# fryzjergda/DesiRNA

Measured on AMD Instinct MI355X. Metric: replica-folds/sec (MFE+PF, L=200, R=64), higher is better.
Workload: dtype int32 (MFE) + f64 (PF); 1 GPU; BASELINE configs[2]: Eterna100-V1 #69 target (L=200), R=64 uniform-random sequences per GPU, -sf Ed-Epf (MFE fill+traceback, PF inside, eval_structure); replicas_per_gpu=64, replicas_total=64, replicas_on_rank0=64, L=200, exchange_every=100, threads_per_workgroup=1024

## Files before the change

### desirna_amd/csrc/fold_common.hpp

```cpp
#pragma once
#include <stdint.h>

#include "tables.hpp"
#ifdef DRNA_PRIMS_HEADER
#include DRNA_PRIMS_HEADER
#else
#include "gfx950_prims.hpp"
#endif

namespace drna {

constexpr int WAVE = 64;
constexpr int MAXN = 2048;
constexpr int PART_ITEMS = 32;

constexpr int GRES = 28;
enum : int { TW_LIVE = 0, TW_BIRTH = 1, TW_KILL = 2, TW_DEAD = 3 };

#ifndef DRNA_SKIP
#define DRNA_SKIP 0
#endif

enum : int { ST_OK = 0, ST_BAD_CHAR = 1, ST_TRACEBACK = 2, ST_PF_RANGE = 3, ST_SYNC = 4 };

struct Ragged {
  const int* idx = nullptr;
  const int* len = nullptr;
  const int* off = nullptr;
  __device__ int seq_of(int b) const { return idx ? idx[b] : b; }
  __device__ int len_of(int r, int L) const { return len ? len[r] : L; }
  __device__ long long off_of(int r, int L) const { return off ? (long long)off[r] : (long long)r * L; }
};

constexpr int DLAG = 10, KEDGE = DLAG - 5;
constexpr int XP = 224;
struct DualLink {
  int* flagA = nullptr;
  int* flagB = nullptr;
  int32_t* xs = nullptr;
  void* xa = nullptr;
  void* xb = nullptr;
  int base = 0;
  int epoch = 0;
};
__device__ __forceinline__ int dual_base(int epoch, int round) { return (int)((((unsigned)epoch * 8u + (unsigned)round) << 10)); }
__device__ __forceinline__ int dual_done(int epoch) { return (int)((((unsigned)epoch * 8u + 7u) << 10) + 1023u); }
__device__ __forceinline__ bool flag_ge(int v, int target) { return (int)((unsigned)v - (unsigned)target) >= 0; }

__device__ __forceinline__ bool wait_flag_wave(const int* flag, int target) {
  SpinClock clk;
  for (;;) {
    if (flag_ge(__builtin_amdgcn_readfirstlane(ld_agent(flag)), target)) return true;
    if (clk.expired()) return false;
    spin_pause();
  }
}

__device__ __forceinline__ int lane_id() { return threadIdx.x & (WAVE - 1); }
__device__ __forceinline__ int wave_id() { return threadIdx.x >> 6; }

__device__ __forceinline__ int wave_min_i32(int v) {
// ... 284 lines not shown
```

### desirna_amd/csrc/fold_mfe_lds.hpp

```cpp
#pragma once
#include "fold_mfe.hpp"

namespace drna {

constexpr int MFE_FAST_NMAX = 200;
enum : int { E_ALL = 0, E_NEAR = 1, E_FAR = 2, E_COARSE = 3 };
constexpr int GSLOTS = 10;

template <int NT>
struct MfeFastSmem : MfeSmemCore<MFE_FAST_NMAX> {
  static constexpr int NW = NT / WAVE;
  static constexpr int RS = MFE_FAST_NMAX + 2;
  static constexpr int TRI = (MFE_FAST_NMAX - 4) * (MFE_FAST_NMAX - 3) / 2;
  static constexpr int NSLOT = 4 * WAVE;
  static constexpr int NL = MFE_FAST_NMAX + 8;
  int fml[TRI + 8];
  int wring[33 * RS];
  int ciring[32 * RS];
  int dml[4 * RS];
  int hpl[MFE_FAST_NMAX + 2];
  int rowoff[MFE_FAST_NMAX + 2];
  int accG[2][NSLOT], accI[2][NSLOT], accK[2][NSLOT];
  static constexpr int XT_STACK = 0, XT_INT11 = 64, XT_MM1N = 64 + 1024, XT_MM23 = 64 + 1024 + 128;
  int xtab[64 + 1024 + 128 + 128];
// ... 484 lines not shown
  for (int k = tid; k < 1024; k += NT) sm.xtab[SM::XT_INT11 + k] = sm.int11[k] - (((k >> 4) & 7) > 2 ? TermAU : 0);
  for (int k = tid; k < 128; k += NT) {
    sm.xtab[SM::XT_MM1N + k] = sm.mm1n[k] - ((k >> 4) > 2 ? TermAU : 0);
    sm.xtab[SM::XT_MM23 + k] = sm.mm23[k] - ((k >> 4) > 2 ? TermAU : 0);
  }
  for (int j = tid; j <= n && j <= TURN + 1; j += NT) sm.f5[j] = 0;
  if (DUAL) {
    drain_vmem();
    __syncthreads();
    if (tid == 0) st_agent(lk.flagA, lk.base + TURN);
  }
  for (int d = TURN + 1 + wave; d < (DUAL ? min(n, PL_D1) : n); d += NW) mfe_pl_row<false>(sm, T, PL, PLX, ld, n, d, lane, TermAU);
  __syncthreads();
  if (aw < 0) {
    const int d = TURN + 1;
    if (d < n) {
      mfe_prepare_tables<NT>(sm, d, tid, ninio, max_ninio, DUAL ? E_NEAR : E_ALL);
      const int cnt = PL[d * ld + ld - 1];
      if (tid < cnt) { sm.plist[d & 1][tid] = PL[d * ld + tid]; sm.xe[d & 1][tid] = PLX[d * ld + tid]; }
      if (tid == 0) { sm.pcnt[d & 1] = cnt; sm.qhead[0] = 0; sm.qhead[1] = 0; }
    }
  }
  __syncthreads();

  if (aw < 0) {
    int32_t* const xw = reinterpret_cast<int32_t*>(lk.xa);
    int32_t* const xf = xw + (MFE_FAST_NMAX + 2) * XP;
    const int32_t* const xk = reinterpret_cast<const int32_t*>(lk.xb);
    const int32_t* const xi = xk + (MFE_FAST_NMAX + 2) * XP;
    int pfK = INF, pfI = INF, fb_s = 0;
    bool have = false;
    if (DUAL) fb_s = __builtin_amdgcn_readfirstlane(ld_agent(lk.flagB));
    int pw[4] = {0, 0, 0, 0}, px[4] = {0, 0, 0, 0}, pw_cnt = 0;
    auto pl_request = [&](const int dn) {
      const int32_t* row = PL + dn * ld;
      const int32_t* rowx = PLX + dn * ld;
      const bool ag = DUAL && dn >= PL_D1;
      pw_cnt = ag ? ld_agent(row + ld - 1) : row[ld - 1];
      const int nch = (n - dn + WAVE - 1) >> 6;
#pragma unroll
      for (int c = 0; c < 4; c++)
        if (c < nch) {
          const int o = min(lane + c * WAVE, ld - 1);
          pw[c] = ag ? ld_agent(row + o) : row[o];
          px[c] = ag ? ld_agent(rowx + o) : rowx[o];
        }
    };
    if (!sweep_stage && wave == w_pl && TURN + 2 < n) pl_request(TURN + 2);
    for (int k = TURN + 1; k <= n; k++) {
      const int d = k - 1;
      if (DUAL && tid == 0 && d - 2 > TURN) st_agent(lk.flagA, lk.base + d - 2);
      int rqK = INF, rqI = INF, rqF = 0;
      bool rq_have = false, rq_on = false;
      if (DUAL && d > TURN) {
        const int i2 = tid + 1 - ((d + 1) >> 1) - off0;
        rq_have = d + 1 < n && d + 1 >= DUAL_D0 && flag_ge(fb_s, lk.base + d + 1);
        rq_on = rq_have && i2 >= 1 && i2 <= n - d - 1;
        rqK = ld_agent(rq_on ? xk + (d + 1) * XP + i2 : lk.flagB);
        rqI = ld_agent(rq_on ? xi + (d + 1) * XP + i2 : lk.flagB);
        rqF = ld_agent(lk.flagB);
      }
      int fx[4];
      if (!sweep_stage && wave == w_pl) {
        if (k + 1 < n) {
          const int dn = k + 1;
          int* dst = sm.plist[dn & 1];
          int* dxe = sm.xe[dn & 1];
#pragma unroll
          for (int c = 0; c < 4; c++)
            if (lane + c * WAVE < MfeFastSmem<NT>::NL) { dst[lane + c * WAVE] = pw[c]; dxe[lane + c * WAVE] = px[c]; }
          if (lane == 0) { sm.pcnt[dn & 1] = pw_cnt; sm.qhead[dn & 1] = 0; }
        }
        if (k + 2 < n) pl_request(k + 2);
      }
      if (!sweep_q5 && wave == w_q5 && k - 3 >= TURN + 2) {
        const int j = k - 3;
        const int nch = (j - TURN - 1 + WAVE - 1) >> 6;
#pragma unroll
        for (int c = 0; c < 4; c++) {
          const int i = lane + 1 + c * WAVE;
          fx[c] = INF;
          if (c < nch && i <= j - TURN - 1) fx[c] = EXT[j * ld + i];
        }
      }
      if (d > TURN) {
        const int ncell = n - d, sh = d >> 1, par = d & 1;
        const int i = tid + 1 - sh - off0;
        const int dv = as_vector(d), dm1v = as_vector(d - 1);
        int bK = pfK, bI = pfI;
        if (DUAL && d >= DUAL_D0) {
          if (!have) {
            if (!sm.sync_fail && !wait_flag_wave(lk.flagB, lk.base + d)) sm.sync_fail = 1;
            const bool on = i >= 1 && i <= ncell;
            bK = on ? ld_agent(xk + d * XP + i) : INF;
            bI = on ? ld_agent(xi + d * XP + i) : INF;
          }
        }
        if (i >= 1 && i <= ncell) {
          const int aG = sm.accG[par][tid];
          const int aI = DUAL ? min(sm.accI[par][tid], bI) : sm.accI[par][tid];
          const int aK = DUAL ? min(sm.accK[par][tid], bK) : sm.accK[par][tid];
          sm.accG[par][tid] = INF; sm.accI[par][tid] = INF; sm.accK[par][tid] = INF;
          const int j = i + d;
          const int t = pair_type(sm.Sp[i], sm.Sp[j]);
          const int tau = t > 2 ? TermAU : 0;
          int c = INF, info = 0, cb = INF;
          if (t) {
            const int ij = t * 16 + sm.S[i + 1] * 4 + sm.S[j - 1];
            c = mfe_hairpin_e(sm, T, sm.hpl[dm1v], i, j, t);
            c = min(c, aI);
            c = min(c, aG + sm.mmI[ij]);
            const int dml = sm.dml[((d - 2) & 3) * RS + i + 1];
            if (dml < HALF)
              c = min(c, dml + MLclosing + MLintern + tau + sm.mmM[rtype_of(t) * 16 + sm.S[j - 1] * 4 + sm.S[i + 1]]);
            if (c >= HALF) c = INF;
            info = (rtype_of(t) << 4) | (sm.S[j + 1] << 2) | sm.S[i - 1];
            cb = c < INF ? c + tau : INF;
          }
          sm.wring[(d & 31) * RS + i] = cb * 256 + info;
          sm.ciring[(d & 31) * RS + i] = c < INF ? c + sm.mmI[info] : INF;
          {
            Wc[d * ld + i] = c * 256 + info;
            EXT[j * ld + i] = c < INF ? c + tau + mfe_extstem(sm, t, i, j, n) : INF;
          }
          int f = INF;
          if (d - 1 > TURN) {
            const int ro1 = sm.rowoff[dm1v];
            const int fa = sm.fml[ro1 + i], fb = sm.fml[ro1 + i - 1];
            if (fa < HALF) f = fa + MLbase;
            if (fb < HALF) f = min(f, fb + MLbase);
          }
          if (c < INF) f = min(f, c + MLintern + tau + sm.mmM[t * 16 + sm.S[i - 1] * 4 + sm.S[j + 1]]);
          const int dec = aK >= HALF ? INF : aK;
          sm.dml[(d & 3) * RS + i] = dec;
          const int fv = min(f, dec);
          sm.fml[sm.rowoff[dv] + i - 1] = fv;
          if (DUAL) {
            st_agent(xw + d * XP + i, cb * 256 + info);
            st_agent(xf + d * XP + i, fv);
          }
        }
      }
      if (k + 1 < n) {
        const bool outer_idle = NB > 3 && (d >> 1) + off0 >= WAVE;
        const int we = outer_idle ? NB - 1 : w_et;
        if (wave == we) mfe_prepare_etab(sm, k + 1, lane, DUAL ? E_NEAR : E_ALL);
      }
      if (!sweep_q5 && wave == w_q5 && k - 3 >= TURN + 2) {
        const int j = k - 3;
        int m = INF;
#pragma unroll
        for (int c = 0; c < 4; c++) {
          const int i = lane + 1 + c * WAVE;
          if (i <= j - TURN - 1 && fx[c] < HALF) m = min(m, sm.f5[i - 1] + fx[c]);
        }
        m = wave_min_i32_lane63(m);
        const int prev = sm.f5[j - 1];
        if (lane == WAVE - 1) sm.f5[j] = prev < m ? prev : m;
      }
      bool stored = false;
      if (d > TURN) { const int i_ = tid + 1 - (d >> 1) - off0; stored = __ballot(i_ >= 1 && i_ <= n - d) != 0ull; }
      if (DUAL && d > TURN) {
        pfK = rq_on ? rqK : INF; pfI = rq_on ? rqI : INF;
        have = rq_have;
        fb_s = __builtin_amdgcn_readfirstlane(rqF);
      }
      if (stored) stores_in_flight<DUAL ? 4 : 2>(); else stores_in_flight<0>();
      lds_barrier();
    }
  } else {
    int GE[TSL_M], GO[TSL_M];
#pragma unroll
    for (int r = 0; r < TSL_M; r++) { GE[r] = INF; if (TWO_PAR) GO[r] = INF; }
    const int e_bulge1 = keep_i32(T.bulge[1]), e_int23 = keep_i32(T.interior[5] + ninio);
    const int blk_ord = my_tb < 0 ? 0 : my_tb == 0 ? 0 : my_tb == NBT - 1 ? min(1, NBT - 1) : my_tb + 1;
    const int n_free = NA - (TWO_PAR ? 2 : 4) * NBT;
    auto item_rank_of = [&](const int par) -> int {
      if (TWO_PAR) return aw;
      if (my_tb < 0) return aw - 4 * NBT;
      const bool rests = !((my_pm >> par) & 1);
      return n_free + (rests ? 0 : 2 * NBT) + 2 * blk_ord + my_sig;
    };

    int sw[4] = {0, 0, 0, 0}, sx[4] = {0, 0, 0, 0}, sw_cnt = 0;
    auto st_request = [&](const int dn) {
      const int32_t* row = PL + dn * ld;
      const int32_t* rowx = PLX + dn * ld;
      const bool ag = DUAL && dn >= PL_D1;
      sw_cnt = ag ? ld_agent(row + ld - 1) : row[ld - 1];
      const int nch = (n - dn + WAVE - 1) >> 6;
#pragma unroll
      for (int c = 0; c < 4; c++)
        if (c < nch) {
          const int o = min(lane + c * WAVE, ld - 1);
          sw[c] = ag ? ld_agent(row + o) : row[o];
          sx[c] = ag ? ld_agent(rowx + o) : rowx[o];
        }
    };
    if (stager && ((my_pm >> ((TURN + 1) & 1)) & 1) && TURN + 2 < n) st_request(TURN + 2);
    for (int k = TURN + 1; k <= n; k++) {
      if (q5er && !((my_pm >> (k & 1)) & 1) && k - 3 >= TURN + 2) {
        const int j = k - 3;
        const int nch = (j - TURN - 1 + WAVE - 1) >> 6;
        int fx[4];
#pragma unroll
        for (int c = 0; c < 4; c++) {
          const int i = lane + 1 + c * WAVE;
          fx[c] = INF;
          if (c < nch && i <= j - TURN - 1) fx[c] = EXT[j * ld + i];
        }
        int m = INF;
#pragma unroll
        for (int c = 0; c < 4; c++) {
          const int i = lane + 1 + c * WAVE;
          if (i <= j - TURN - 1 && fx[c] < HALF) m = min(m, sm.f5[i - 1] + fx[c]);
        }
        m = wave_min_i32_lane63(m);
        const int prev = sm.f5[j - 1];
        if (lane == WAVE - 1) sm.f5[j] = prev < m ? prev : m;
      }
// ... 145 lines not shown
```

### desirna_amd/csrc/fold_pf_lds.hpp

```cpp
#pragma once
#include <cstddef>
#include "eval_structure.hpp"
#include "fold_pf.hpp"

namespace drna {

constexpr int PF_FAST_NMAX = 200;
constexpr int PGSLOTS = 10;
constexpr int PNG = 3;
constexpr int TSL = 14;

template <int NT>
struct PfFastSmem {
  static constexpr int NW = NT / WAVE;
  static constexpr int RS = PF_FAST_NMAX + 2;
  static constexpr int NSLOT = 4 * WAVE;
  static constexpr int NL = PF_FAST_NMAX + 8;
  double qbi[32 * RS];
  double dring[4 * RS];
  double qm1row[2][RS];
  double urow[2][RS];
  double hpw[PF_FAST_NMAX + 2];
  double q5[PF_FAST_NMAX + 2];
  double partG[2][2][NSLOT];
// ... 106 lines not shown
  for (int q = Q1 - 1; q >= Q0; q--) {
    const int s = 4 + SIG + 2 * q;
    if (s > 30) continue;
    G[q] = q > 0 ? fma3_f64(a[q - Q0] + b[q - Q0], c[q - Q0].x, G[q - 1]) : (a[q - Q0] + b[q - Q0]) * c[q - Q0].x;
    acc += G[q] * c[q - Q0].y;
  }
}

template <class SM, int SIG>
__device__ __forceinline__ double pf_tower2_step(const SM& sm, double (&G)[TSL], int dv, int i8) {
  const int cbase = as_vector((int)(reinterpret_cast<const char*>(&sm.twc[0][0]) - reinterpret_cast<const char*>(sm.qbi)));
  double acc0 = 0.0, acc1 = 0.0, acc2 = 0.0;
  pf_tower2_part<SM, SIG, 9, 14>(sm, G, dv, i8, cbase, acc0);
  pf_tower2_part<SM, SIG, 4, 9>(sm, G, dv, i8, cbase, acc1);
  pf_tower2_part<SM, SIG, 0, 4>(sm, G, dv, i8, cbase, acc2);
  return (acc0 + acc1) + acc2;
}


#ifndef DRNA_PKE
#define DRNA_PKE 5
#endif
constexpr int PKE = DRNA_PKE;
constexpr int KT_NL = PKE + 3;
constexpr int KT_U = (2 * KT_NL + 3) / 4;
constexpr int KT_BMIN = (12 + 2 * PKE + 3) / 4;
constexpr int KT_D0 = 4 * KT_BMIN - 3;
constexpr int KT_MF = (4 * ((PF_FAST_NMAX - 1) / 4) - 11 - 2 * PKE + 15) / 16;
constexpr int KT_DEPTH = 3;
static_assert(PKE >= 4, "a tile's operands must be final when the first of its four steps comes");

__device__ __forceinline__ void kt_near_counts(int i, int d, int& nl, int& nh) {
  const int j = i + d, a = (i - 1) >> 2, c = (j - 1) >> 2, tot = max(d - 2 * TURN - 2, 0);
  if (c - a >= KT_BMIN) { nl = 4 * a + 4 + PKE - i; nh = j - 4 * c - 1 + PKE; }
  else { nl = min(tot, KT_NL); nh = tot - nl; }
}
__device__ __forceinline__ bool kt_has_far(int i, int d) { return ((i + d - 1) >> 2) - ((i - 1) >> 2) >= KT_BMIN; }

template <typename RS>
__device__ __forceinline__ void k_near_row(RS rs, int tab8, int ld, int d, int i, int row, double& v0, double& v1) {
  int nl0, nh0, nl1, nh1;
  kt_near_counts(i, d, nl0, nh0);
  kt_near_counts(i + 1, d, nl1, nh1);
  f64x2 a[KT_U], c[KT_U];
#pragma unroll
  for (int u = 0; u < KT_U; u++) {
    const int s = row + 4 * u, y = s - KT_NL;
    const bool low = s < KT_NL;
    const bool ok0 = low ? s < nl0 : y < nh0, ok1 = low ? s < nl1 : y < nh1;
    int tt = low ? TURN + 1 + s : d - TURN - 2 - y;
    tt = (ok0 || ok1) ? tt : TURN + 1;
    a[u] = buf_load_f64x2(rs, (tt * ld + i) * 8, 0);
    c[u] = buf_load_f64x2(rs, tab8 + ((d - tt - 1) * ld + i + tt + 1) * 8, 0);
    if (!ok0) a[u].x = 0.0;
    if (!ok1) a[u].y = 0.0;
  }
  double p0 = 0.0, p1 = 0.0, q0 = 0.0, q1 = 0.0;
#pragma unroll
  for (int u = 0; u < KT_U; u++) {
    if (u & 1) { p1 = fma(a[u].x, c[u].x, p1); q1 = fma(a[u].y, c[u].y, q1); }
    else { p0 = fma(a[u].x, c[u].x, p0); q0 = fma(a[u].y, c[u].y, q0); }
  }
  v0 = p0 + p1; v1 = q0 + q1;
}

constexpr int KT_PRE = 3;
struct KTile {
  double al, bl, av[KT_PRE], bv[KT_PRE];
  int vA, vB;
  int a, c, last;
  bool mask_last;
};
template <bool SC1, typename RS>
__device__ __forceinline__ void k_tile_issue(RS rs, int tab8, int ld, int n, int a, int B, int lane, KTile& t) {
  const int c = a + B, m_lo = 4 * a + 9 + PKE, m_hi = 4 * c - 3 - PKE;
  const int last = __builtin_amdgcn_readfirstlane((m_hi - m_lo + 16) >> 4) - 1;
  const int q = lane & 3, moff = (lane & 12) + (lane >> 4);
  const int i = 4 * a + 1 + q, jc = min(4 * c + 1 + q, n);
  const int sA = 16 * ld * 8, sB = 16 * (ld - 1) * 8;
  const int m0 = m_lo + moff, ml = min(m0 + 16 * last, m_hi);
  const int vA = (i - (1 + i) * ld + m0 * ld) * 8;
  const int vB = tab8 + (jc * ld - (m0 + 16 * last) * (ld - 1)) * 8;
  const int vAl = (i - (1 + i) * ld + ml * ld) * 8, vBl = tab8 + (jc * ld - ml * (ld - 1)) * 8;
  t.a = a; t.c = c; t.last = last; t.mask_last = m0 + 16 * last > m_hi; t.vA = vA; t.vB = vB;
#pragma unroll
  for (int u = 0; u < KT_PRE; u++) {
    if (u < last) {
      t.av[u] = SC1 ? buf_load_f64_aux(rs, vA, u * sA) : buf_load_f64(rs, vA, u * sA);
      t.bv[u] = SC1 ? buf_load_f64_aux(rs, vB, (last - u) * sB) : buf_load_f64(rs, vB, (last - u) * sB);
    }
  }
  t.al = SC1 ? buf_load_f64_aux(rs, vAl, 0) : buf_load_f64(rs, vAl, 0);
  t.bl = SC1 ? buf_load_f64_aux(rs, vBl, 0) : buf_load_f64(rs, vBl, 0);
}
template <bool SC1, typename RS, typename ST>
__device__ __forceinline__ void k_tile_finish(RS rs, int ld, const KTile& t, int n, int lane, ST store) {
  const int sA = 16 * ld * 8, sB = 16 * (ld - 1) * 8, last = t.last;
  double acc0 = 0.0, acc1 = 0.0;
#pragma unroll
  for (int u = 0; u < KT_PRE; u++) {
    if (u < last) {
      if (u & 1) acc1 = mfma_f64_4x4x4_4b(t.av[u], t.bv[u], acc1);
      else acc0 = mfma_f64_4x4x4_4b(t.av[u], t.bv[u], acc0);
    }
  }
#pragma unroll
  for (int u0 = KT_PRE; u0 < KT_MF - 1; u0 += KT_DEPTH) {
    if (u0 < last) {
// ... 54 lines not shown
  const int ld = A.ld, tid = threadIdx.x, lane = lane_id();
  const int wave = __builtin_amdgcn_readfirstlane(wave_id());
  double* base = A.ws + (long long)r * A.ws_stride;
  const long long tab = (long long)ld * ld;
  double* DFAR = base + 5 * tab;
  const auto rsX = __builtin_amdgcn_make_buffer_rsrc((void*)base, (short)0, (int)(2 * tab * 8), 0x00020000);
  const int* flagA = A.hflags + (long long)r * 64;
  int* flagB = A.hflags + (long long)r * 64 + 32;
  int* ctl = reinterpret_cast<int*>(&sm);
  if (tid == 0) ctl[0] = 0;
  if (EV.n_targets > 0) {
    constexpr int NEV = NW < 8 ? NW : 8;
    EvalSmem* es = reinterpret_cast<EvalSmem*>(ctl + 32);
    if (wave < NEV)
      for (int k = wave; k < EV.n_targets; k += NEV) eval_one(es[wave], EV, r, k, lane);
  }
  {
    const char* seq = A.seqs + A.rg.off_of(r, n);
    for (int k = tid; k < n; k += NT) { const int c = enc_nt(seq[k]); sm.S[k + 1] = (unsigned char)(c < 0 ? 0 : c); }
    if (tid == 0) { sm.S[0] = 0; sm.S[n + 1] = 0; }
    __syncthreads();
    int32_t* PL = reinterpret_cast<int32_t*>(base + 4 * tab);
    for (int d = PFL_D1 + wave; d < n; d += NW) pf_pl_row<true>(sm, PL, ld, n, d, lane);
    drain_vmem();
  }
  __syncthreads();
  if (tid == 0) st_agent(flagB, A.hbase + KT_D0 - 1);
  const int Bmax = (n - 1) >> 2;
  for (int B = KT_BMIN; B <= Bmax; B++) {
    if (wave == 0) {
      int seen = 0;
      const bool ok = strip_wait(flagA, A.hbase, 4 * B - 5 - PKE, seen);
      if (lane == 0 && (!ok || seen == A.hbase + STRIP_DONE)) ctl[0] = 1;
    }
    __syncthreads();
    if (ctl[0]) break;
    if (!(DRNA_SKIP & 8))
      for (int a = wave; a <= Bmax - B; a += NW) {
        KTile t;
        k_tile_issue<true>(rsX, (int)tab * 8, ld, n, a, B, lane, t);
        k_tile_finish<true>(rsX, ld, t, n, lane, [&](int d, int i, double v) { st_agent(&DFAR[d * ld + i], v); });
      }
    drain_vmem();
    __syncthreads();
    if (tid == 0) st_agent(flagB, A.hbase + (B == Bmax ? n : 4 * B));
  }
}

template <int NT, bool TILES = true>
__device__ __forceinline__ void pf_lds_body(PfFastSmem<NT>& sm, PfArgs A, const EvalArgs& EV, int bx_in = -1, int helper_in = -1) {
  constexpr int NW = NT / WAVE;
  constexpr int RS = PfFastSmem<NT>::RS;
  const PfTables& T = *A.T;
  const bool hm = A.helper != 0;
  const int bx = bx_in >= 0 ? bx_in : hm ? blockIdx.x >> 1 : blockIdx.x;
  const bool is_helper = hm && (helper_in >= 0 ? helper_in != 0 : (blockIdx.x & 1) != 0);
  const int r = A.rg.seq_of(bx);
  A.L = A.rg.len_of(r, A.L);
  const int n = A.L, ld = A.ld;
  if (is_helper) {
    if (A.helper == 2) return;
    pf_kfar_helper<NT>(A, EV, sm, r, n);
    return;
  }
  const int tid = threadIdx.x, lane = lane_id();
  const int wave = __builtin_amdgcn_readfirstlane(wave_id());

  double* base = A.ws + (long long)r * A.ws_stride;
  const long long tab = (long long)ld * ld;
  double* QM = base + 2 * tab;
  double* QM1 = base + 3 * tab;
  int32_t* PL = reinterpret_cast<int32_t*>(base + 4 * tab);
  double* QEXT = base + 6 * tab;

  const double eTau = T.TermAU, eMLc = T.MLclosing, eMLi = T.MLintern;
  const double b1 = A.eMLb[1], sc1 = A.scale[1], sc2 = A.scale[2];

  stage_energy_tables<NT>(sm, T, tid);
  for (int k = tid; k < 128; k += NT) {
    const double inv = 1.0 / T.mmI[k];
    sm.rinv[k] = inv;
    sm.rbul[k] = ((k >> 4) > 2 ? eTau : 1.0) * inv;
    sm.r1n[k] = T.mm1n[k] * inv;
    sm.r23[k] = T.mm23[k] * inv;
  }
  for (int k = tid; k <= n; k += NT) sm.hpw[k] = A.hp_w[k];
  for (int t = tid; t < 36; t += NT) {
    sm.eWt[t][0] = t >= 2 && t <= 30 ? T.bulge[t] * A.scale[t + 2] : 0.0;
    sm.eWt[t][1] = t >= 4 && t <= 30 ? T.interior[t] * T.eninio[t - 2] * A.scale[t + 2] : 0.0;
  }
  if (tid == 0) {
    sm.xc[0] = T.bulge[1] * A.scale[3]; sm.xc[1] = T.interior[5] * T.eninio[1] * A.scale[7];
    sm.xc[2] = A.scale[4]; sm.xc[3] = A.scale[5]; sm.xc[4] = A.scale[6];
    sm.xc[8] = eTau; sm.xc[9] = eMLc; sm.xc[10] = eMLi; sm.xc[11] = b1; sm.xc[12] = sc2;
  }
  for (int k = tid; k < 32; k += NT) {
    sm.twc[k][0] = k >= 4 && k <= 30 ? T.eninio[k - 4] : 0.0;
    sm.twc[k][1] = k >= 6 && k <= 30 ? T.interior[k] * A.scale[k + 2] : 0.0;
  }
  for (int k = tid; k < 4 * RS; k += NT) sm.dring[k] = 0.0;
  for (int k = tid; k < 32 * RS; k += NT) { sm.qbi[k] = 0.0; sm.info[k] = 0; }
  for (int k = tid; k < 2 * RS; k += NT) { (&sm.qm1row[0][0])[k] = 0.0; (&sm.urow[0][0])[k] = 0.0; }
  for (int k = tid; k < 2 * 2 * PfFastSmem<NT>::NSLOT; k += NT) (&sm.partG[0][0][0])[k] = 0.0;
  for (int k = tid; k < 2 * 4 * PfFastSmem<NT>::NSLOT; k += NT) (&sm.partK[0][0][0])[k] = 0.0;
  for (int k = tid; k < 2 * PfFastSmem<NT>::NSLOT; k += NT) (&sm.accE[0][0])[k] = 0.0;
  for (int k = tid; k < 6 * PfFastSmem<NT>::NSLOT; k += NT) (&sm.accX[0][0][0])[k] = 0.0;
  if (tid == 0) sm.q5[0] = 1.0;
// ... 10 lines not shown

  const int NB = (n + WAVE - 1) / WAVE;
  const int off0 = (NB * WAVE - n) / 2;
  const int aw = wave - NB;
  constexpr bool TWO_PAR = NT < 1024;
  const int nT = n - 10, NBT = nT > 0 ? (nT + WAVE - 1) / WAVE : 0;
  const int T0 = max(0, off0 + 5 - (NBT * WAVE - nT) / 2);
  int my_tb = -1, my_sig = 0, my_pm = 0;
  if (aw >= 0) {
    if (TWO_PAR) { if (aw < 2 * NBT) { my_tb = aw >> 1; my_sig = aw & 1; my_pm = 3; } }
    else if (aw < 4 * NBT) { my_tb = aw >> 2; const int x = (aw + my_tb) & 3; my_sig = x & 1; my_pm = 1 << (x >> 1); }
  }
  const int w_pl = NB > 2 ? 2 : 0, w_q5 = NB - 1;

  if (aw < 0) {
    const int d = TURN + 1;
    if (d < n) {
      const int cnt = PL[d * ld + ld - 1];
      if (tid < cnt) sm.plist[d & 1][tid] = PL[d * ld + tid];
      if (tid == 0) { sm.pcnt[d & 1] = cnt; sm.qhead[0] = 0; sm.qhead[1] = 0; sm.qtile[0] = 0; sm.qtile[1] = 0; }
    }
  }
  __syncthreads();


  const auto rsQ = __builtin_amdgcn_make_buffer_rsrc((void*)QM, (short)0, (int)(2 * tab * 8), 0x00020000);


  double* XQM = base, *XQM1 = base + tab, *DFAR = base + 5 * tab;
  int* flagA = hm ? A.hflags + (long long)r * 64 : nullptr;
  const int* flagB = hm ? A.hflags + (long long)r * 64 + 32 : nullptr;
  double dfar_cur = 0.0, dfar_next = 0.0;
  int fb_last = 0;
  bool helper_lost = false, pl_seen = false;
  auto run_items = [&](const int d) {
    const int ncell = n - d, sh = d >> 1, par = d & 1;
    const int slot0 = sh + off0 - 1;
    const int pcnt = __builtin_amdgcn_readfirstlane(sm.pcnt[par]);
    const int nblk = (ncell + 31) >> 5;
    const int nK = ((DRNA_SKIP & 8) || d < 2 * TURN + 3) ? 0 : nblk;
    const int nE = (DRNA_SKIP & 2) ? 0 : (pcnt + 3) >> 2, nX = (DRNA_SKIP & 4) ? 0 : 3 * ((pcnt + WAVE - 1) / WAVE);
    const int nItems = __builtin_amdgcn_readfirstlane(nK + nE + nX);
    for (int it0 = queue_pop(&sm.qhead[par], lane); it0 < nItems; it0 = queue_pop(&sm.qhead[par], lane)) {
      const int it = it0 < nX ? nK + nE + it0 : it0 - nX;
      if (it < nK) {
        const int blk = it, cl = lane & 15, row = lane >> 4;
        int i = (blk << 5) + 2 * cl + 1;
        const bool act0 = i <= ncell, act1 = i + 1 <= ncell;
        i = act0 ? i : 1;
        double v0, v1;
        k_near_row(rsQ, (int)tab * 8, ld, d, i, row, v0, v1);
        if (act0) sm.partK[par][row][i + slot0] = v0;
        if (act1) sm.partK[par][row][i + 1 + slot0] = v1;
      } else if (it < nK + nE) {
        const int q = 4 * (it - nK) + (lane >> 4);
        const int pe = sm.plist[par][q < pcnt ? q : pcnt - 1];
        const int i0 = pe & 255, ij = pe >> 8;
        const int tA = (lane & 15) + 2, tBr = tA + 16, tB = tBr > 30 ? 30 : tBr;
        const f64x2 wA = *reinterpret_cast<const f64x2*>(&sm.eWt[tA][0]), wB = *reinterpret_cast<const f64x2*>(&sm.eWt[tBr][0]);
        const int oA = ((d - 2 - tA) & 31) * RS + i0, oB = ((d - 2 - tB) & 31) * RS + i0;
        const double a1 = sm.qbi[oA + 1], a2 = sm.qbi[oA + 2], a3 = sm.qbi[oA + tA], a4 = sm.qbi[oA + tA + 1];
        const double b1_ = sm.qbi[oB + 1], b2_ = sm.qbi[oB + 2], b3_ = sm.qbi[oB + tB], b4_ = sm.qbi[oB + tB + 1];
        const int fa1 = sm.info[oA + 1], fa2 = sm.info[oA + 2], fa3 = sm.info[oA + tA], fa4 = sm.info[oA + tA + 1];
        const int fb1 = sm.info[oB + 1], fb2 = sm.info[oB + 2], fb3 = sm.info[oB + tB], fb4 = sm.info[oB + tB + 1];
        const double ra1 = sm.rbul[fa1], ra4 = sm.rbul[fa4], ra2 = sm.r1n[fa2], ra3 = sm.r1n[fa3];
        const double rb1 = sm.rbul[fb1], rb4 = sm.rbul[fb4], rb2 = sm.r1n[fb2], rb3 = sm.r1n[fb3];
        const double bul = (a1 * ra1 + a4 * ra4) * wA.x + (b1_ * rb1 + b4_ * rb4) * wB.x;
        const double one = (a2 * ra2 + a3 * ra3) * wA.y + (b2_ * rb2 + b3_ * rb3) * wB.y;
        double v = bul * ((ij >> 4) > 2 ? sm.xc[as_vector(8)] : 1.0) + one * sm.mm1n[ij];
        v = dpp_add_f64<0x111, 0xF>(v);
        v = dpp_add_f64<0x112, 0xF>(v);
        v = dpp_add_f64<0x114, 0xF>(v);
        v = dpp_add_f64<0x118, 0xF>(v);
        if ((lane & 15) == 15 && q < pcnt) sm.accE[par][i0 + slot0] = v;
      } else {
        const int xi = it - nK - nE;
        const int ch = xi / 3, grp = xi - 3 * ch;
        const int q = ch * WAVE + lane;
        const int pe = sm.plist[par][q < pcnt ? q : pcnt - 1];
        const int i = pe & 255, cxv = pe >> 8, t = cxv >> 4, si1 = (cxv >> 2) & 3, sj1 = cxv & 3;
        double sum;
        if (grp == 0) {
          double w[4];
          int f[4];
#pragma unroll
          for (int shp = 0; shp < 4; shp++) {
            const int u1 = shp >> 1, u2 = shp == 1 || shp == 3 ? 1 : 0;
            const int dp = d - 2 - u1 - u2;
            const int off = (dp & 31) * RS + 1 + u1 + i;
            w[shp] = dp > TURN ? sm.qbi[off] : 0.0;
            f[shp] = dp > TURN ? sm.info[off] : 0;
          }
          sum = w[0] * sm.rinv[f[0]] * sm.stack[t * 8 + (f[0] >> 4)] * sm.xc[as_vector(12)];
          sum += (w[1] * sm.rinv[f[1]] * sm.stack[t * 8 + (f[1] >> 4)] + w[2] * sm.rinv[f[2]] * sm.stack[t * 8 + (f[2] >> 4)]) * sm.xc[as_vector(0)];
          sum += w[3] * sm.rinv[f[3]] * sm.int11[(t * 8 + (f[3] >> 4)) * 16 + si1 * 4 + sj1] * sm.xc[as_vector(2)];
        } else if (grp == 1) {
          const int dpa = d - 5, dpb = d - 6;
          const int oa = (dpa & 31) * RS + 2 + i, ob = (dpa & 31) * RS + 3 + i, oc = (dpb & 31) * RS + 3 + i;
          const double wa = dpa > TURN ? sm.qbi[oa] : 0.0, wb = dpa > TURN ? sm.qbi[ob] : 0.0, wc = dpb > TURN ? sm.qbi[oc] : 0.0;
          const int fa = dpa > TURN ? sm.info[oa] : 0, fb = dpa > TURN ? sm.info[ob] : 0, fc = dpb > TURN ? sm.info[oc] : 0;
          const double ga = T.int21[(t * 8 + (fa >> 4)) * 64 + si1 * 16 + ((fa >> 2) & 3) * 4 + sj1];
          const double gb = T.int21[((fb >> 4) * 8 + t) * 64 + ((fb >> 2) & 3) * 16 + si1 * 4 + (fb & 3)];
          const double gc = T.int22[(t * 8 + (fc >> 4)) * 256 + si1 * 64 + (fc & 3) * 16 + ((fc >> 2) & 3) * 4 + sj1];
          sum = (wa * sm.rinv[fa] * ga + wb * sm.rinv[fb] * gb) * sm.xc[as_vector(3)] + wc * sm.rinv[fc] * gc * sm.xc[as_vector(4)];
        } else {
          const int dp = d - 7;
          const int oa = (dp & 31) * RS + 3 + i, ob = (dp & 31) * RS + 4 + i;
          const double wa = dp > TURN ? sm.qbi[oa] : 0.0, wb = dp > TURN ? sm.qbi[ob] : 0.0;
          const int fa = dp > TURN ? sm.info[oa] : 0, fb = dp > TURN ? sm.info[ob] : 0;
          sum = (wa * sm.r23[fa] + wb * sm.r23[fb]) * sm.mm23[cxv] * sm.xc[as_vector(1)];
        }
        if (q < pcnt) sm.accX[par][grp][i + slot0] = sum;
      }
    }
  };

  auto run_tiles = [&](const int d) {
    const int Bmax = (n - 1) >> 2, Bt = ((d + 3) >> 2) + 1, ph = (d + 3) & 3;
    if (!TILES || (DRNA_SKIP & 8) || hm || Bt < KT_BMIN || Bt > Bmax) return;
    const int cnt = Bmax - Bt + 1, per = (cnt + 3) >> 2, a0 = ph * per;
    const int nT = __builtin_amdgcn_readfirstlane(max(0, min(cnt, a0 + per) - a0));
    for (int it = queue_pop(&sm.qtile[d & 1], lane); it < nT; it = queue_pop(&sm.qtile[d & 1], lane)) {
      KTile t;
      k_tile_issue<false>(rsQ, (int)tab * 8, ld, n, a0 + it, Bt, lane, t);
      k_tile_finish<false>(rsQ, ld, t, n, lane, [&](int dd, int ii, double v) { DFAR[dd * ld + ii] = v; });
    }
  };

  if (aw < 0) {
    double fTau = sm.xc[as_vector(8)], fMLc = sm.xc[as_vector(9)], fMLi = sm.xc[as_vector(10)], fb1 = sm.xc[as_vector(11)], fsc2 = sm.xc[as_vector(12)];
    int pl_cnt = 0, pl0 = 0, pl1 = 0, pl2 = 0, pl3 = 0;
    auto pl_request = [&](const int dn) {
      const int32_t* row = PL + dn * ld;
      if (hm && dn >= PFL_D1) {
        if (!pl_seen) {
          int seen = 0;
          if (!helper_lost && !flag_ge(fb_last, A.hbase + KT_D0 - 1) && !strip_wait(flagB, A.hbase, KT_D0 - 1, seen)) { sm.flag = 2; helper_lost = true; }
          pl_seen = true;
        }
        pl_cnt = ld_agent(row + ld - 1);
        pl0 = ld_agent(row + lane); pl1 = ld_agent(row + lane + WAVE); pl2 = ld_agent(row + lane + 2 * WAVE);
        pl3 = ld_agent(row + min(lane + 3 * WAVE, ld - 1));
      } else {
        pl_cnt = row[ld - 1];
        pl0 = row[lane]; pl1 = row[lane + WAVE]; pl2 = row[lane + 2 * WAVE]; pl3 = row[min(lane + 3 * WAVE, ld - 1)];
      }
    };
    if (wave == w_pl && TURN + 2 < n) pl_request(TURN + 2);
    for (int k = TURN + 1; k <= n; k++) {
      const int d = k - 1;
      if (wave == w_pl) {
        if (k + 1 < n) {
          int* dst = sm.plist[(k + 1) & 1];
          dst[lane] = pl0; dst[lane + WAVE] = pl1; dst[lane + 2 * WAVE] = pl2;
          if (lane + 3 * WAVE < PfFastSmem<NT>::NL) dst[lane + 3 * WAVE] = pl3;
          if (lane == 0) { sm.pcnt[(k + 1) & 1] = pl_cnt; sm.qhead[(k + 1) & 1] = 0; sm.qtile[(k + 1) & 1] = 0; }
        }
        if (k + 2 < n) pl_request(k + 2);
      }
      const bool job_q5 = wave == w_q5 && k - 3 >= TURN + 2;
      double qx0 = 0.0, qx1 = 0.0, qx2 = 0.0, qx3 = 0.0;
      if (job_q5) {
        const int j = k - 3, top = j - TURN - 1;
        const double* col = QEXT + j * ld;
        qx0 = lane + 1 <= top ? col[lane + 1] : 0.0;
        qx1 = lane + 1 + WAVE <= top ? col[lane + 1 + WAVE] : 0.0;
        qx2 = lane + 1 + 2 * WAVE <= top ? col[lane + 1 + 2 * WAVE] : 0.0;
        qx3 = lane + 1 + 3 * WAVE <= top ? col[lane + 1 + 3 * WAVE] : 0.0;
      }
      int f_req = 0;
      double d_req = 0.0;
      dfar_cur = dfar_next;
      if (hm) {
        if (tid == 0 && k - 2 > TURN) st_agent(flagA, A.hbase + (k - 2));
        f_req = ld_agent(flagB);
        if (k >= KT_D0 && k < n && !helper_lost && !flag_ge(fb_last, A.hbase + k)) {
          int seen = 0;
          if (!strip_wait(flagB, A.hbase, k, seen)) { sm.flag = 2; helper_lost = true; }
        }
      }
      if (k >= KT_D0 && k < n) {
        const int ic = tid + 1 - (k >> 1) - off0;
        if (ic >= 1 && ic <= n - k && kt_has_far(ic, k)) d_req = hm ? ld_agent(&DFAR[k * ld + ic]) : DFAR[k * ld + ic];
      }
      if (d > TURN) {
        const int ncell = n - d, sh = d >> 1, par = d & 1;
        const int i = tid + 1 - sh - off0;
        if (i >= 1 && i <= ncell) {
          const int j = i + d;
          const int si = sm.S[i], sj = sm.S[j], si1 = sm.S[i + 1],
                    sj1 = sm.S[j - 1], sim = sm.S[i - 1], sjp = sm.S[j + 1];
          const double aG = d >= 10 ? sm.partG[par][0][tid] + sm.partG[par][1][tid] : 0.0;
          const double aKn = d >= 2 * TURN + 3 ? (sm.partK[par][0][tid] + sm.partK[par][1][tid]) + (sm.partK[par][2][tid] + sm.partK[par][3][tid]) : 0.0;
          const double aK = aKn + dfar_cur;
          const int t = pair_type(si, sj);
          const double cTau = fTau, cMLc = fMLc, cMLi = fMLi, cb1 = fb1, csc2 = fsc2;
          const double tau = t > 2 ? cTau : 1.0;
          const int ij = t * 16 + si1 * 4 + sj1, rt = rtype_of(t);
          const int info = t ? (rt << 4) | (sjp << 2) | sim : 0;
          const double aE = sm.accE[par][tid], aX = (sm.accX[par][0][tid] + sm.accX[par][1][tid]) + sm.accX[par][2][tid];
          const double wH = sm.mmH[ij], wI = sm.mmI[ij], wMc = sm.mmM[rt * 16 + sj1 * 4 + si1], wInfo = sm.mmI[info];
          const double dprev = sm.dring[((d - 2) & 3) * RS + i + 1];
          const int ex = t * 16 + sim * 4 + sjp;
          const double wExt = sm.mmExt[ex], wMs = sm.mmM[ex], w5 = sm.d5[t * 4 + sim], w3 = sm.d3[t * 4 + sjp];
          const int pp = (d - 1) & 1;
          const double m1p = sm.qm1row[pp][i], m1q = sm.qm1row[pp][i + 1], up = sm.urow[pp][i + 1];
          double qb = 0.0;
          if (t) {
            const int u = d - 1;
            double hp;
            if (u == 3 || u == 4 || u == 6) {
              int code = 0;
              const int len = u + 2;
              for (int q = 0; q < len; q++) code |= sm.S[i + q] << (2 * q);
              hp = -1.0;
              if (u == 3) { for (int q = 0; q < T.n_tri; q++) if (T.tri_code[q] == code) hp = T.tri_w[q] * A.scale[u + 2]; if (hp < 0.0) hp = sm.hpw[u] * tau; }
              else if (u == 4) { for (int q = 0; q < T.n_tetra; q++) if (T.tetra_code[q] == code) hp = T.tetra_w[q] * A.scale[u + 2]; }
              else { for (int q = 0; q < T.n_hexa; q++) if (T.hexa_code[q] == code) hp = T.hexa_w[q] * A.scale[u + 2]; }
              if (hp < 0.0) hp = sm.hpw[u] * wH;
            } else {
              hp = sm.hpw[u] * wH;
            }
            qb = hp + aE + aX + aG * wI;
            qb += dprev * cMLc * cMLi * tau * wMc * csc2;
          }
          sm.qbi[(d & 31) * RS + i] = qb * wInfo;
          sm.info[(d & 31) * RS + i] = (unsigned char)info;
          const double me = (i > 1 && j < n) ? wExt : i > 1 ? w5 : j < n ? w3 : 1.0;
          const double mm = (i > 1 && j < n) ? wMs : i > 1 ? w5 : j < n ? w3 : 1.0;
          const double ext = t ? qb * tau * me : 0.0, stem = t ? qb * cMLi * tau * mm : 0.0;
          const double m1 = m1p * cb1 + stem;
          const double U = cb1 * (m1q + up);
          sm.qm1row[par][i] = m1;
          sm.urow[par][i] = U;
          sm.dring[(d & 3) * RS + i] = aK;
          {
            QEXT[j * ld + i] = ext;
            QM1[d * ld + i] = m1;
            QM[d * ld + i] = m1 + aK + U;
            if (hm) { st_agent(&XQM1[d * ld + i], m1); st_agent(&XQM[d * ld + i], m1 + aK + U); }
          }
        }
      }
      if (job_q5) {
        const int j = k - 3, top = j - TURN - 1;
        double sq = 0.0;
        if (lane + 1 <= top) sq += sm.q5[lane] * qx0;
        if (lane + 1 + WAVE <= top) sq += sm.q5[lane + WAVE] * qx1;
        if (lane + 1 + 2 * WAVE <= top) sq += sm.q5[lane + 2 * WAVE] * qx2;
        if (lane + 1 + 3 * WAVE <= top) sq += sm.q5[lane + 3 * WAVE] * qx3;
        sq = wave_total_f64_lane63(sq);
        if (lane == WAVE - 1) sm.q5[j] = sm.q5[j - 1] * sc1 + sq;
      }
      if (k < n) run_items(k);
      dfar_next = d_req;
      if (hm) fb_last = __builtin_amdgcn_readfirstlane(f_req);
      __syncthreads();
    }
  } else {
    double GE[TSL], GO[TSL];
#pragma unroll
    for (int q = 0; q < TSL; q++) { GE[q] = 0.0; if (TWO_PAR) GO[q] = 0.0; }
    for (int k = TURN + 1; k <= n; k++) {
      if (k < n) {
        const int d = k;
        const int ncell = n - d, sh = d >> 1, par = d & 1;
        const int lo = sh + off0, hi = ncell + sh + off0 - 1;

        if (!(DRNA_SKIP & 1) && ((my_pm >> par) & 1) && d >= 10) {
          const int blo = T0 + my_tb * WAVE;
          int i = blo + lane + 1 - sh - off0;
          i = i < 1 ? 1 : (i > ncell ? ncell : i);
          const int dv = as_vector(d + 30), i8 = i * 8;
          if (blo <= hi && blo + WAVE - 1 >= lo) {
            double accG = 0.0;
            if constexpr (TWO_PAR) {
              if (par) accG = my_sig ? pf_tower2_step<PfFastSmem<NT>, 1>(sm, GO, dv, i8) : pf_tower2_step<PfFastSmem<NT>, 0>(sm, GO, dv, i8);
            }
            if (!TWO_PAR || !par) accG = my_sig ? pf_tower2_step<PfFastSmem<NT>, 1>(sm, GE, dv, i8) : pf_tower2_step<PfFastSmem<NT>, 0>(sm, GE, dv, i8);
            sm.partG[par][my_sig][T0 + my_tb * WAVE + lane] = accG;
          }
        }
        run_tiles(d);
        run_items(d);
      }
      __syncthreads();
    }
  }

  const int jq0 = max(TURN + 2, n - 2);
  if (NW >= 3) {
    if (wave < 3 && jq0 + wave <= n) {
      const int j = jq0 + wave;
      double sq = 0.0;
      for (int i = lane + 1; i <= j - TURN - 1; i += WAVE) sq += sm.q5[i - 1] * QEXT[j * ld + i];
      sq = wave_total_f64_lane63(sq);
      if (lane == WAVE - 1) sm.xc[13 + wave] = sq;
    }
    __syncthreads();
    if (tid == 0)
      for (int j = jq0; j <= n; j++) sm.q5[j] = sm.q5[j - 1] * sc1 + sm.xc[13 + j - jq0];
    __syncthreads();
  } else if (wave == 0) {
    for (int j = jq0; j <= n; j++) pf_q5_column<NT>(sm, QEXT, ld, j, lane, sc1);
  }
  if (wave == 0) {
    if (lane == 0) {
      const double Z = sm.q5[n];
      if (!(Z > 0.0) || !(Z < 1.0e300)) {
        A.status[r] = ST_PF_RANGE;
// ... 24 lines not shown
```

Baseline: 151,900 replica-folds/s.

## Make global stores unconditional and replace full barriers with LDS-only barriers in helper mode

In both the MFE and PF LDS kernels, the per-diagonal global stores in helper/dual mode now happen unconditionally outside the cell-active branch: inactive lanes write to a dummy index 0, so the stores are issued uniformly. Asm-based 'take_over' fences pin prefetched agent loads so the compiler schedules them early. Full __syncthreads plus store waits are replaced by an LDS-only barrier, with a single vmem drain on the last iteration. In the PF kernel, helper mode is forced on for the non-tiled path and the helper flag is signalled one diagonal later. The MFE hairpin energy for longer loops is simplified to a table lookup. All of this is meant to let global-memory traffic overlap with compute across diagonals, at the risk of ordering bugs and of writing garbage values to slot 0.

```diff
diff --git a/desirna_amd/csrc/fold_common.hpp b/desirna_amd/csrc/fold_common.hpp
--- a/desirna_amd/csrc/fold_common.hpp
+++ b/desirna_amd/csrc/fold_common.hpp
@@ -7,6 +7,20 @@
 #else
 #include "gfx950_prims.hpp"
 #endif
+
+namespace drna {
+#ifdef DRNA_PRIMS_HEADER
+inline void issue_fence() {}
+template <typename T> inline void take_over(T&) {}
+template <typename T, typename U> inline void take_over(T&, U&) {}
+template <typename T, typename U, typename V> inline void take_over(T&, U&, V&) {}
+#else
+__device__ __forceinline__ void issue_fence() { __builtin_amdgcn_sched_barrier(0); }
+template <typename T> __device__ __forceinline__ void take_over(T& x) { asm volatile("" : "+v"(x)); }
+template <typename T, typename U> __device__ __forceinline__ void take_over(T& x, U& y) { asm volatile("" : "+v"(x), "+v"(y)); }
+template <typename T, typename U, typename V> __device__ __forceinline__ void take_over(T& x, U& y, V& z) { asm volatile("" : "+v"(x), "+v"(y), "+v"(z)); }
+#endif
+}
 
 namespace drna {
 
diff --git a/desirna_amd/csrc/fold_mfe_lds.hpp b/desirna_amd/csrc/fold_mfe_lds.hpp
--- a/desirna_amd/csrc/fold_mfe_lds.hpp
+++ b/desirna_amd/csrc/fold_mfe_lds.hpp
@@ -560,7 +560,7 @@
       if (DUAL && tid == 0 && d - 2 > TURN) st_agent(lk.flagA, lk.base + d - 2);
       int rqK = INF, rqI = INF, rqF = 0;
       bool rq_have = false, rq_on = false;
-      if (DUAL && d > TURN) {
+      if (DUAL) {
         const int i2 = tid + 1 - ((d + 1) >> 1) - off0;
         rq_have = d + 1 < n && d + 1 >= DUAL_D0 && flag_ge(fb_s, lk.base + d + 1);
         rq_on = rq_have && i2 >= 1 && i2 <= n - d - 1;
@@ -591,6 +591,7 @@
           if (c < nch && i <= j - TURN - 1) fx[c] = EXT[j * ld + i];
         }
       }
+      int o_wc = 0, o_ext = 0, o_xw = 0, o_xf = 0;
       if (d > TURN) {
         const int ncell = n - d, sh = d >> 1, par = d & 1;
         const int i = tid + 1 - sh - off0;
@@ -602,6 +603,7 @@
             const bool on = i >= 1 && i <= ncell;
             bK = on ? ld_agent(xk + d * XP + i) : INF;
             bI = on ? ld_agent(xi + d * XP + i) : INF;
+            take_over(bK, bI);
           }
         }
         if (i >= 1 && i <= ncell) {
@@ -615,7 +617,8 @@
           int c = INF, info = 0, cb = INF;
           if (t) {
             const int ij = t * 16 + sm.S[i + 1] * 4 + sm.S[j - 1];
-            c = mfe_hairpin_e(sm, T, sm.hpl[dm1v], i, j, t);
+            if (d - 1 > 6) c = sm.hpl[dm1v] + sm.mmH[ij];
+            else { c = mfe_hairpin_e(sm, T, sm.hpl[dm1v], i, j, t); take_over(c); }
             c = min(c, aI);
             c = min(c, aG + sm.mmI[ij]);
             const int dml = sm.dml[((d - 2) & 3) * RS + i + 1];
@@ -628,8 +631,9 @@
           sm.wring[(d & 31) * RS + i] = cb * 256 + info;
           sm.ciring[(d & 31) * RS + i] = c < INF ? c + sm.mmI[info] : INF;
           {
-            Wc[d * ld + i] = c * 256 + info;
-            EXT[j * ld + i] = c < INF ? c + tau + mfe_extstem(sm, t, i, j, n) : INF;
+            const int wc = c * 256 + info, ext = c < INF ? c + tau + mfe_extstem(sm, t, i, j, n) : INF;
+            if (DUAL) { o_wc = wc; o_ext = ext; }
+            else { Wc[d * ld + i] = wc; EXT[j * ld + i] = ext; }
           }
           int f = INF;
           if (d - 1 > TURN) {
@@ -643,11 +647,17 @@
           sm.dml[(d & 3) * RS + i] = dec;
           const int fv = min(f, dec);
           sm.fml[sm.rowoff[dv] + i - 1] = fv;
-          if (DUAL) {
-            st_agent(xw + d * XP + i, cb * 256 + info);
-            st_agent(xf + d * XP + i, fv);
-          }
-        }
+          if (DUAL) { o_xw = cb * 256 + info; o_xf = fv; }
+        }
+      }
+      if (DUAL) {
+        const int i = tid + 1 - (d >> 1) - off0;
+        const bool on = d > TURN && i >= 1 && i <= n - d;
+        const int is = on ? i : 0, js = on ? i + d : d;
+        Wc[d * ld + is] = o_wc;
+        EXT[js * ld + is] = o_ext;
+        st_agent(xw + d * XP + is, o_xw);
+        st_agent(xf + d * XP + is, o_xf);
       }
       if (k + 1 < n) {
         const bool outer_idle = NB > 3 && (d >> 1) + off0 >= WAVE;
@@ -666,14 +676,17 @@
         const int prev = sm.f5[j - 1];
         if (lane == WAVE - 1) sm.f5[j] = prev < m ? prev : m;
       }
-      bool stored = false;
-      if (d > TURN) { const int i_ = tid + 1 - (d >> 1) - off0; stored = __ballot(i_ >= 1 && i_ <= n - d) != 0ull; }
-      if (DUAL && d > TURN) {
+      if (DUAL) {
+        take_over(rqK, rqI, rqF);
         pfK = rq_on ? rqK : INF; pfI = rq_on ? rqI : INF;
         have = rq_have;
         fb_s = __builtin_amdgcn_readfirstlane(rqF);
-      }
-      if (stored) stores_in_flight<DUAL ? 4 : 2>(); else stores_in_flight<0>();
+      } else {
+        bool stored = false;
+        if (d > TURN) { const int i_ = tid + 1 - (d >> 1) - off0; stored = __ballot(i_ >= 1 && i_ <= n - d) != 0ull; }
+        if (stored) stores_in_flight<2>(); else stores_in_flight<0>();
+      }
+      if (k == n) drain_vmem();
       lds_barrier();
     }
   } else {
diff --git a/desirna_amd/csrc/fold_pf_lds.hpp b/desirna_amd/csrc/fold_pf_lds.hpp
--- a/desirna_amd/csrc/fold_pf_lds.hpp
+++ b/desirna_amd/csrc/fold_pf_lds.hpp
@@ -182,8 +182,14 @@
     tt = (ok0 || ok1) ? tt : TURN + 1;
     a[u] = buf_load_f64x2(rs, (tt * ld + i) * 8, 0);
     c[u] = buf_load_f64x2(rs, tab8 + ((d - tt - 1) * ld + i + tt + 1) * 8, 0);
-    if (!ok0) a[u].x = 0.0;
-    if (!ok1) a[u].y = 0.0;
+  }
+  issue_fence();
+#pragma unroll
+  for (int u = 0; u < KT_U; u++) {
+    const int s = row + 4 * u, y = s - KT_NL;
+    const bool low = s < KT_NL;
+    if (!(low ? s < nl0 : y < nh0)) a[u].x = 0.0;
+    if (!(low ? s < nl1 : y < nh1)) a[u].y = 0.0;
   }
   double p0 = 0.0, p1 = 0.0, q0 = 0.0, q1 = 0.0;
 #pragma unroll
@@ -344,7 +350,7 @@
   constexpr int NW = NT / WAVE;
   constexpr int RS = PfFastSmem<NT>::RS;
   const PfTables& T = *A.T;
-  const bool hm = A.helper != 0;
+  const bool hm = !TILES || A.helper != 0;
   const int bx = bx_in >= 0 ? bx_in : hm ? blockIdx.x >> 1 : blockIdx.x;
   const bool is_helper = hm && (helper_in >= 0 ? helper_in != 0 : (blockIdx.x & 1) != 0);
   const int r = A.rg.seq_of(bx);
@@ -461,6 +467,7 @@
         k_near_row(rsQ, (int)tab * 8, ld, d, i, row, v0, v1);
         if (act0) sm.partK[par][row][i + slot0] = v0;
         if (act1) sm.partK[par][row][i + 1 + slot0] = v1;
+        take_over(v0, v1);
       } else if (it < nK + nE) {
         const int q = 4 * (it - nK) + (lane >> 4);
         const int pe = sm.plist[par][q < pcnt ? q : pcnt - 1];
@@ -555,7 +562,10 @@
         pl0 = row[lane]; pl1 = row[lane + WAVE]; pl2 = row[lane + 2 * WAVE]; pl3 = row[min(lane + 3 * WAVE, ld - 1)];
       }
     };
-    if (wave == w_pl && TURN + 2 < n) pl_request(TURN + 2);
+    if (wave == w_pl && TURN + 2 < n) {
+      pl_request(TURN + 2);
+      take_over(pl_cnt, pl0, pl1); take_over(pl2, pl3);
+    }
     for (int k = TURN + 1; k <= n; k++) {
       const int d = k - 1;
       if (wave == w_pl) {
@@ -581,7 +591,7 @@
       double d_req = 0.0;
       dfar_cur = dfar_next;
       if (hm) {
-        if (tid == 0 && k - 2 > TURN) st_agent(flagA, A.hbase + (k - 2));
+        if (tid == 0 && k - 3 > TURN) st_agent(flagA, A.hbase + (k - 3));
         f_req = ld_agent(flagB);
         if (k >= KT_D0 && k < n && !helper_lost && !flag_ge(fb_last, A.hbase + k)) {
           int seen = 0;
@@ -592,6 +602,7 @@
         const int ic = tid + 1 - (k >> 1) - off0;
         if (ic >= 1 && ic <= n - k && kt_has_far(ic, k)) d_req = hm ? ld_agent(&DFAR[k * ld + ic]) : DFAR[k * ld + ic];
       }
+      double o_ext = 0.0, o_m1 = 0.0, o_qm = 0.0;
       if (d > TURN) {
         const int ncell = n - d, sh = d >> 1, par = d & 1;
         const int i = tid + 1 - sh - off0;
@@ -643,13 +654,20 @@
           sm.qm1row[par][i] = m1;
           sm.urow[par][i] = U;
           sm.dring[(d & 3) * RS + i] = aK;
-          {
-            QEXT[j * ld + i] = ext;
-            QM1[d * ld + i] = m1;
-            QM[d * ld + i] = m1 + aK + U;
-            if (hm) { st_agent(&XQM1[d * ld + i], m1); st_agent(&XQM[d * ld + i], m1 + aK + U); }
-          }
+          const double qm = m1 + aK + U;
+          if (hm) { o_ext = ext; o_m1 = m1; o_qm = qm; }
+          else { QEXT[j * ld + i] = ext; QM1[d * ld + i] = m1; QM[d * ld + i] = qm; }
         }
+      }
+      if (hm) {
+        const int i = tid + 1 - (d >> 1) - off0;
+        const bool on = d > TURN && i >= 1 && i <= n - d;
+        const int is = on ? i : 0, js = on ? i + d : d;
+        QEXT[js * ld + is] = o_ext;
+        QM1[d * ld + is] = o_m1;
+        QM[d * ld + is] = o_qm;
+        st_agent(&XQM1[d * ld + is], o_m1);
+        st_agent(&XQM[d * ld + is], o_qm);
       }
       if (job_q5) {
         const int j = k - 3, top = j - TURN - 1;
@@ -662,9 +680,16 @@
         if (lane == WAVE - 1) sm.q5[j] = sm.q5[j - 1] * sc1 + sq;
       }
       if (k < n) run_items(k);
-      dfar_next = d_req;
-      if (hm) fb_last = __builtin_amdgcn_readfirstlane(f_req);
-      __syncthreads();
+      if (hm) {
+        take_over(d_req, f_req);
+        dfar_next = d_req;
+        fb_last = __builtin_amdgcn_readfirstlane(f_req);
+        if (k == n) drain_vmem();
+        lds_barrier();
+      } else {
+        dfar_next = d_req;
+        __syncthreads();
+      }
     }
   } else {
     double GE[TSL], GO[TSL];
```

New measurement: 151,800 replica-folds/s. No clear change (-0.0%).
